# TEAM-AIOLY/OCM-VAE-SIMCA

Measured on AMD Instinct MI355X. Metric: spectra/sec SIMCA fit+Q/T² score at 1M×2048, higher is better.
Workload: dtype f32

## Files before the change

### ocm-vae-simca_amd/csrc/ocm_gram.hip

```cpp
#include <cstring>
#include <string>
#include <type_traits>
#include <vector>

#include "ocm_gram_map.h"
#include "ocm_internal.h"

namespace {

__device__ __forceinline__ float load_y(const float* __restrict__ X, int64_t ldx, int64_t r, int col, int p,
                                        const PrepArgs& pa) {
  if (pa.w == 0 && !pa.snv) return X[r * ldx + col];
  float m = 0.f, sc = 1.f;
  if (pa.snv) {
    m = pa.rowstat[2 * r];
    sc = pa.rowstat[2 * r + 1];
  }
  return ocm::prep_elem(X + r * ldx, p, col, pa, m, sc);
}


constexpr int MAXSEG = 32;

struct SegTable {
  int64_t begin[MAXSEG + 1];
  int32_t cprefix[MAXSEG + 1];
  int32_t nseg;
  int32_t chunk_rows;
};

__device__ __forceinline__ void tile_coords(int t, int nt, int& ti, int& tj) {
  ti = 0;
  while (t >= nt - ti) {
    t -= nt - ti;
    ++ti;
  }
  tj = ti + t;
}

template <int GT, int BK_>
struct GramCfg {
  static constexpr int BK = BK_;
  static constexpr int WN = GT / 64;
  static constexpr int THREADS = 2 * WN * 64;
  static constexpr int MT = GT / 64;
  static constexpr int C4 = GT / 4;
  static constexpr int RSTEP = THREADS / C4;
  static constexpr int LPP = BK / RSTEP;
};

constexpr int GATHER_MAX_CHUNK = 2048;

template <int GT, int BK_, bool VEC, bool GATHER>
__global__ __launch_bounds__(GT * 2, 2) void k_gram(
    const float* __restrict__ X, int64_t ldx, const int64_t* __restrict__ rows, int p, const float* __restrict__ shift,
    SegTable st, int nt, int ntiles, int total_wg, float* __restrict__ part, double* __restrict__ colpart) {
  using Cfg = GramCfg<GT, BK_>;
  constexpr int BK = Cfg::BK, MT = Cfg::MT, LPP = Cfg::LPP, RSTEP = Cfg::RSTEP;
  __shared__ __attribute__((aligned(16))) float lds[2][2][BK][GT];
  __shared__ int64_t ridx[GATHER ? GATHER_MAX_CHUNK : 1];

  const int b = blockIdx.x;
  const int q8 = total_wg / 8, r8 = total_wg % 8, x8 = b % 8;
  const int wg = (x8 < r8 ? x8 * (q8 + 1) : r8 * (q8 + 1) + (x8 - r8) * q8) + b / 8;
  const int chunk = wg / ntiles;
  const int tile = wg - chunk * ntiles;
  int ti, tj;
  tile_coords(tile, nt, ti, tj);
  const bool diag = (ti == tj);
  const int I = ti * GT, J = tj * GT;

  int s = 0;
  while (s + 1 < st.nseg && chunk >= st.cprefix[s + 1]) ++s;
  const int64_t r0 = st.begin[s] + (int64_t)(chunk - st.cprefix[s]) * st.chunk_rows;
  const int64_t r1 = min(r0 + (int64_t)st.chunk_rows, st.begin[s + 1]);
  const int nstage = (int)((r1 - r0 + BK - 1) / BK);

  const int tid = threadIdx.x;
  const int lane = tid & 63, wave = tid >> 6;
  const int wm = wave / Cfg::WN, wn = wave % Cfg::WN;
  if (GATHER) {
// ... 484 lines not shown
      }
    }
    if (tid < p)
      for (int r = 0; r < nr; ++r) csum += ys[r][tid];
  }
#pragma unroll
  for (int u = 0; u < MAXPT; ++u) {
    const int e = tid + 256 * u;
    if (e < npair) part[(size_t)blockIdx.x * npair + e] = acc[u];
  }
  if (tid < p) cpart[(size_t)blockIdx.x * p + tid] = csum;
}

__global__ __launch_bounds__(256) void k_gram_small_reduce(const double* __restrict__ part,
                                                           const double* __restrict__ cpart, int p, int c0, int c1,
                                                           double* __restrict__ G, double* __restrict__ colsum) {
  const int e = blockIdx.x * 256 + threadIdx.x;
  const int npair = p * (p + 1) / 2;
  if (e < npair) {
    int i = 0, rem = e;
    while (rem >= p - i) {
      rem -= p - i;
      ++i;
    }
    const int j = i + rem;
    double v = 0.0;
    for (int c = c0; c < c1; ++c) v += part[(size_t)c * npair + e];
    G[(size_t)i * p + j] = v;
    G[(size_t)j * p + i] = v;
  }
  if (e < p) {
    double v = 0.0;
    for (int c = c0; c < c1; ++c) v += cpart[(size_t)c * p + e];
    colsum[e] = v;
  }
}

typedef int i32x4 __attribute__((ext_vector_type(4)));
typedef int i32x16 __attribute__((ext_vector_type(16)));
constexpr int Q8T = 128, Q8K = 32, Q8BLK = 1536, Q8SPB = Q8BLK / Q8K;
constexpr float Q8BASE = 254.f;

struct Q8Plan {
  char* digits;
  size_t plane;
  float* scale;
  int P8;
  int nblk;
  const float* thr;
  uint32_t* flags;
  int fw;
  uint32_t* nmark;
};

constexpr float Q8TAU = 16.f;
constexpr int Q8GROUP = 32;

__device__ __forceinline__ uint32_t q8_byte(float a, int u) { return ((uint32_t)(int)a & 0xffu) << (8 * u); }

__device__ __forceinline__ uint32_t q8_pack4(float a0, float a1, float a2, float a3) {
  const uint32_t lo = __builtin_amdgcn_perm((uint32_t)(int)a1, (uint32_t)(int)a0, 0x0c0c0400u);
  const uint32_t hi = __builtin_amdgcn_perm((uint32_t)(int)a3, (uint32_t)(int)a2, 0x04000c0cu);
  return lo | hi;
}

__device__ __forceinline__ int q8_qslot(int P) { return P ^ ((P >> 3) & 7); }

constexpr int Q8QC = 32;
constexpr int Q8QS = Q8BLK / 16;
constexpr int Q8QT = Q8QS * (Q8QC / 4);
struct Q8TailLds {
  union {
    struct {
      __attribute__((aligned(16))) float wmax[Q8QS][Q8QC];
      __attribute__((aligned(16))) double wsum[Q8QS][Q8QC];
      float pmax[8][Q8QC];
      double psum[8][Q8QC];
    } r;
    __attribute__((aligned(16))) char stage[3 * Q8SPB * Q8QC * 32];
  } u;
  __attribute__((aligned(16))) float fmax_[Q8QC];
};
__device__ __forceinline__ void q8_tail(f32x4 (&v)[16], int tid, int cq, int rs, int cg0, int c0, int64_t rb,
                                        const Q8Plan& q, int chunk, int b, const SegTable& st,
                                        double* __restrict__ colblk, Q8TailLds& L, const f32x4 th) {
  constexpr int QC = Q8QC, NT = Q8QT;
  char* stage = L.u.stage;
  auto& wmax = L.u.r.wmax;
  auto& wsum = L.u.r.wsum;
  auto& pmax = L.u.r.pmax;
  auto& psum = L.u.r.psum;
  float* fmax_ = L.fmax_;
#ifdef OCM_Q8_DIAG_COPY
  (void)wsum; (void)wmax; (void)pmax; (void)psum; (void)fmax_; (void)th; (void)colblk; (void)c0;
  i32x4 w[3][4];
#pragma unroll
  for (int dg = 0; dg < 3; ++dg)
#pragma unroll
    for (int e = 0; e < 4; ++e)
#pragma unroll
      for (int k = 0; k < 4; ++k)
        w[dg][e][k] = (int)(__builtin_bit_cast(uint32_t, v[4 * k][e]) ^ __builtin_bit_cast(uint32_t, v[4 * k + 1][e]) ^
                            __builtin_bit_cast(uint32_t, v[4 * k + 2][e]) ^ __builtin_bit_cast(uint32_t, v[4 * k + 3][e])) + dg;
#else
  double cs[4] = {0.0, 0.0, 0.0, 0.0};
#pragma unroll
// ... 585 lines not shown
      const bool mi = (m >> (ty >> 3)) & 1u;
      const bool mj = (m >> (2 + (tx >> 3))) & 1u;
      if (!(mi || mj)) continue;
#pragma unroll
      for (int a = 0; a < 4; ++a) {
        const double u = yi[r][4 * ty + a];
#pragma unroll
        for (int b = 0; b < 4; ++b) acc[a][b] = fma(u, yj[r][4 * tx + b], acc[a][b]);
      }
    }
  }
  double* Gs = G + (size_t)seg * p * p;
#pragma unroll
  for (int a = 0; a < 4; ++a)
#pragma unroll
    for (int b = 0; b < 4; ++b) {
      const int gi = I + 4 * ty + a, gj = J + 4 * tx + b;
      if (gi >= p || gj >= p) continue;
      Gs[(size_t)gi * p + gj] += acc[a][b];
      if (ti != tj) Gs[(size_t)gj * p + gi] += acc[a][b];
    }
}

__global__ __launch_bounds__(256, 1) void k_gram8d(Q8Plan q, SegTable st, int nt, int ntiles, int total_wg,
                                                   int nwg, int nblocks, float* __restrict__ part) {
  __shared__ __attribute__((aligned(16))) float scl[4][2 * 64];
  __shared__ __attribute__((aligned(16))) float runl[4][4][4][64][4];

  const int wg = ocm_g8::logical_item(total_wg, blockIdx.x);
  const int chunk = wg / nwg;
  const int wave = __builtin_amdgcn_readfirstlane(threadIdx.x >> 6);
  const int bi = (wg - chunk * nwg) * 4 + wave;
  if (bi >= nblocks) return;
  int ti = -1, tj = 0, wm = 0, wn = 0;
  {
    int rem = bi;
    for (int u = 0; u < nt && ti < 0; u += ocm_g8::BAND_R)
      for (int v = u; v < nt && ti < 0; v += ocm_g8::BAND_C)
        for (int a = u; a < min(nt, u + ocm_g8::BAND_R) && ti < 0; ++a)
          for (int c = max(v, a); c < min(nt, v + ocm_g8::BAND_C); ++c) {
            const int nbk = (a == c) ? 3 : 4;
            if (rem < nbk) {
              ti = a;
              tj = c;
              wm = (a == c) ? (rem == 2) : (rem >> 1);
              wn = (a == c) ? (rem >= 1) : (rem & 1);
              break;
            }
            rem -= nbk;
          }
  }
  const int tile = ti * nt - ti * (ti - 1) / 2 + (tj - ti);
  const int I = ti * Q8T, J = tj * Q8T;
  int s = 0;
  while (s + 1 < st.nseg && chunk >= st.cprefix[s + 1]) ++s;
  const int64_t r0 = st.begin[s] + (int64_t)(chunk - st.cprefix[s]) * st.chunk_rows;
  const int64_t r1 = min(r0 + (int64_t)st.chunk_rows, st.begin[s + 1]);
  const int nb = (int)((r1 - r0 + Q8BLK - 1) / Q8BLK);
  const int nstage3 = nb * Q8SPB;
  const size_t gbase = (size_t)chunk * (st.chunk_rows / Q8K);

  const int lane = threadIdx.x & 63;
  const int l31 = lane & 31, h = lane >> 5;
  const size_t gstride = (size_t)q.P8 * 32;
  const uint32_t span = (uint32_t)((size_t)nstage3 * gstride);
  const char* cbase = q.digits + gbase * gstride;
  __amdgpu_buffer_rsrc_t ra[3], rb[3];
#pragma unroll
  for (int dg = 0; dg < 3; ++dg) {
    ra[dg] = __builtin_amdgcn_make_buffer_rsrc((void*)(cbase + dg * q.plane + (size_t)(I + wm * 64) * 32), 0, span,
                                               0x00020000);
    rb[dg] = __builtin_amdgcn_make_buffer_rsrc((void*)(cbase + dg * q.plane + (size_t)(J + wn * 64) * 32), 0, span,
                                               0x00020000);
  }
  const int voff = l31 * 32 + h * 16;
  const float* srow = q.scale + (size_t)chunk * q.nblk * q.P8 + I + wm * 64 + lane;
  const float* scol = q.scale + (size_t)chunk * q.nblk * q.P8 + J + wn * 64 + lane;

#define Q8D_LOAD(FA, FB, STG)                                                                         \
  do {                                                                                              \
    const int so_ = (STG) * (int)gstride;                                                           \
    _Pragma("unroll") for (int x_ = 0; x_ < 2; ++x_)                                                \
    _Pragma("unroll") for (int dg_ = 0; dg_ < 3; ++dg_) {                                           \
      FA[x_][dg_] = (i32x4)__builtin_amdgcn_raw_buffer_load_b128(ra[dg_], voff + x_ * 1024, so_, 0); \
      FB[x_][dg_] = (i32x4)__builtin_amdgcn_raw_buffer_load_b128(rb[dg_], voff + x_ * 1024, so_, 0); \
    }                                                                                               \
  } while (0)
  i32x16 acc1[2][2], acc2[2][2], acc3[2][2];
#pragma unroll
  for (int a = 0; a < 2; ++a)
#pragma unroll
    for (int c = 0; c < 2; ++c) {
      acc1[a][c] = i32x16{};
      acc2[a][c] = i32x16{};
      acc3[a][c] = i32x16{};
#pragma unroll
      for (int g = 0; g < 4; ++g)
        *reinterpret_cast<f32x4*>(&runl[wave][a * 2 + c][g][lane][0]) = f32x4{0.f, 0.f, 0.f, 0.f};
    }
  float SR = 0.f, SC = 0.f;
  auto flush = [&]() __attribute__((always_inline)) {
    constexpr float w2 = 1.f / 254.f, w3 = 1.f / (254.f * 254.f);
    scl[wave][lane] = SR;
    scl[wave][64 + lane] = SC;
#pragma unroll
    for (int a = 0; a < 2; ++a) {
#pragma unroll
      for (int c = 0; c < 2; ++c) {
        const float sj = scl[wave][64 + c * 32 + l31];
#pragma unroll
        for (int g = 0; g < 4; ++g) {
          const f32x4 si = *reinterpret_cast<const f32x4*>(&scl[wave][a * 32 + 8 * g + 4 * h]);
          f32x4* rp = reinterpret_cast<f32x4*>(&runl[wave][a * 2 + c][g][lane][0]);
          f32x4 rv = *rp;
#pragma unroll
          for (int e = 0; e < 4; ++e) {
            const int r = 4 * g + e;
            const float v = fmaf((float)acc3[a][c][r], w3, fmaf((float)acc2[a][c][r], w2, (float)acc1[a][c][r]));
            rv[e] = fmaf(v, si[e] * sj, rv[e]);
          }
          *rp = rv;
        }
        __builtin_amdgcn_sched_barrier(0);
      }
    }
  };
  auto step_il = [&](i32x4 (&CA)[2][3], i32x4 (&CB)[2][3], i32x4 (&NA)[2][3], i32x4 (&NB)[2][3], int stg,
                     bool z) __attribute__((always_inline)) {
    const int so_ = min(stg + 2, nstage3 - 1) * (int)gstride;
#pragma unroll
// ... 73 lines not shown
#endif
constexpr int G8P_TMAP = 2048;
template <bool SKIP>
__global__ __launch_bounds__(256, 1) void k_gram8e(Q8Plan q, SegTable st, int nt, int ntiles, int total_wg,
                                                   int nwg, int nblocks, float* __restrict__ part, int chunk0,
                                                   int map) {
  __shared__ __attribute__((aligned(16))) float scl[4][2 * 64];
  __shared__ __attribute__((aligned(16))) float runl[4][16][64][4];
  __shared__ uint16_t tmap[G8P_TMAP];

  const int noffr = ntiles - nt;
  const bool tabled = noffr <= G8P_TMAP;
  if (tabled) {
    for (int r = threadIdx.x; r < noffr; r += 256) {
      int a, c;
      ocm_g8::offdiag_tile(nt, r, a, c);
      tmap[r] = (uint16_t)(a << 8 | c);
    }
    __syncthreads();
  }
  const ocm_g8::Slot sl = ocm_g8::map_slot(map, total_wg, (int)gridDim.x, (int)blockIdx.x);
  if (sl.count == 0) return;

  const int wave = __builtin_amdgcn_readfirstlane(threadIdx.x >> 6);
  const int lane = threadIdx.x & 63;
  const int l15 = lane & 15, g4 = lane >> 4;
  constexpr int SPB = Q8BLK / 64;
  const size_t gstride = (size_t)q.P8 * 32;
  const int voff = (g4 >> 1) * (int)gstride + l15 * 32 + (g4 & 1) * 16;
  const int sstride = 2 * (int)gstride;
  const int vout = (4 * g4 * Q8T + l15) * 4;
  constexpr uint32_t OUT_SPAN = (63 * Q8T + 64) * 4;

  struct Item {
    __amdgpu_buffer_rsrc_t ra[3], rb[3];
    __amdgpu_buffer_rsrc_t rout;
    const float *srow, *scol;
    int nb, nvs;
  };
  auto setup = [&](int wg) __attribute__((always_inline)) -> Item {
    const int cl = wg / nwg, chunk = chunk0 + cl;
    ocm_g8::Block k = ocm_g8::block_of(nt, ntiles, nblocks, wg - cl * nwg, wave);
    if (k.offrank >= 0) {
      if (tabled) {
        const int v = __builtin_amdgcn_readfirstlane((int)tmap[k.offrank]);
        k.ti = v >> 8;
        k.tj = v & 255;
      } else {
        ocm_g8::offdiag_tile(nt, k.offrank, k.ti, k.tj);
      }
    }
    const int tile = ocm_g8::tile_index(nt, k.ti, k.tj);
    const int I = k.ti * Q8T + k.wm * 64, J = k.tj * Q8T + k.wn * 64;
    int s = 0;
    while (s + 1 < st.nseg && chunk >= st.cprefix[s + 1]) ++s;
    const int64_t r0 = st.begin[s] + (int64_t)(chunk - st.cprefix[s]) * st.chunk_rows;
    const int64_t r1 = min(r0 + (int64_t)st.chunk_rows, st.begin[s + 1]);
    Item it;
    it.nb = (int)((r1 - r0 + Q8BLK - 1) / Q8BLK);
    it.nvs = SKIP ? (int)((r1 - r0 + 63) / 64) : it.nb * SPB;
    const size_t gbase = (size_t)chunk * (st.chunk_rows / Q8K);
    const uint32_t span = (uint32_t)((size_t)it.nb * Q8SPB * gstride);
    const char* cbase = q.digits + gbase * gstride;
#pragma unroll
    for (int dg = 0; dg < 3; ++dg) {
      it.ra[dg] = __builtin_amdgcn_make_buffer_rsrc((void*)(cbase + dg * q.plane + (size_t)I * 32), 0, span, 0x00020000);
      it.rb[dg] = __builtin_amdgcn_make_buffer_rsrc((void*)(cbase + dg * q.plane + (size_t)J * 32), 0, span, 0x00020000);
    }
    it.srow = q.scale + (size_t)chunk * q.nblk * q.P8 + I;
    it.scol = q.scale + (size_t)chunk * q.nblk * q.P8 + J;
    float* out = part + ((size_t)chunk * ntiles + tile) * (Q8T * Q8T) + k.wm * 64 * Q8T + k.wn * 64;
    it.rout = __builtin_amdgcn_make_buffer_rsrc((void*)out, 0, k.dead ? 0u : OUT_SPAN, 0x00020000);
    return it;
  };

  i32x4 acc1[4][4], acc2[4][4], acc3[4][4];
  float SR = 0.f, SC = 0.f;
  auto flush = [&](bool first) __attribute__((always_inline)) {
    constexpr float w2 = 1.f / 254.f, w3 = 1.f / (254.f * 254.f);
    scl[wave][lane] = SR;
    scl[wave][64 + lane] = SC;
#pragma unroll
    for (int a = 0; a < 4; ++a) {
      const f32x4 si = *reinterpret_cast<const f32x4*>(&scl[wave][a * 16 + 4 * g4]);
#pragma unroll
      for (int c = 0; c < 4; ++c) {
        const float sj = scl[wave][64 + c * 16 + l15];
        f32x4* rp = reinterpret_cast<f32x4*>(&runl[wave][a * 4 + c][lane][0]);
        f32x4 rv = *rp;
        if (first) rv = f32x4{0.f, 0.f, 0.f, 0.f};
#pragma unroll
        for (int e = 0; e < 4; ++e) {
          const float v = fmaf((float)acc3[a][c][e], w3, fmaf((float)acc2[a][c][e], w2, (float)acc1[a][c][e]));
          rv[e] = fmaf(v, si[e] * sj, rv[e]);
        }
        *rp = rv;
      }
      __builtin_amdgcn_sched_barrier(0);
    }
  };
  auto load_frag = [&](i32x4 (&FA)[4][3], i32x4 (&FB)[4][3], int i, int so, const __amdgpu_buffer_rsrc_t (&da)[3],
                       const __amdgpu_buffer_rsrc_t (&db)[3]) __attribute__((always_inline)) {
    const int grp = i / 3, dg = i % 3;
    if (grp >= 1 && grp <= 4)
      FB[grp - 1][dg] = (i32x4)__builtin_amdgcn_raw_buffer_load_b128(db[dg], voff + (grp - 1) * 512, so, 0);
    else {
      const int x = grp == 0 ? 0 : grp - 4;
      FA[x][dg] = (i32x4)__builtin_amdgcn_raw_buffer_load_b128(da[dg], voff + x * 512, so, 0);
    }
  };
  auto store_sub = [&](const f32x4& pv, int i, __amdgpu_buffer_rsrc_t ro) __attribute__((always_inline)) {
    const int a = i >> 2, c = i & 3;
#pragma unroll
    for (int e = 0; e < 4; ++e)
      __builtin_amdgcn_raw_buffer_store_b32(__builtin_bit_cast(unsigned, (float)pv[e]), ro, vout,
                                            ((a * 16 + e) * Q8T + c * 16) * 4, OCM_G8E_STORE_AUX);
  };
  auto step = [&](i32x4 (&CA)[4][3], i32x4 (&CB)[4][3], i32x4 (&NA)[4][3], i32x4 (&NB)[4][3], int so,
                  const __amdgpu_buffer_rsrc_t (&da)[3], const __amdgpu_buffer_rsrc_t (&db)[3], bool z, bool bar,
                  auto tail, __amdgpu_buffer_rsrc_t ro) __attribute__((always_inline)) {
    constexpr bool TAIL = decltype(tail)::value;
    f32x4 pv = {0.f, 0.f, 0.f, 0.f};
#pragma unroll
// ... 156 lines not shown
      tab.cprefix[s - s0] = cprefix[s] - cprefix[s0];
    }
    const int64_t gchunks = cprefix[s1] - cprefix[s0];
    if (gchunks == 0) continue;
    const int64_t total = gchunks * ntiles;
    OCM_REQUIRE(total < (1LL << 31), "ocm_gram_f32: too many workgroups");
    float* pg = part + (size_t)cprefix[s0] * ntiles * GT * GT;
    double* col_g = colpart + (size_t)cprefix[s0] * nt * GT;
    ocm::TimedRegion tr(ctx, OCM_KERNEL_GRAM, st);
    dim3 grid((unsigned)total), blk(Cfg::THREADS);
#define OCM_GRAM_LAUNCH(V_, G_)                                                                                    \
  hipLaunchKernelGGL((k_gram<GT, BK, V_, G_>), grid, blk, 0, st, X, ldx, rows, p, shift, tab, nt, ntiles, (int)total, \
                     pg, col_g)
    if (split3) {
      if (rows)
        hipLaunchKernelGGL(k_gram3<true>, grid, dim3(G3THREADS), 0, st, X, ldx, rows, p, shift, tab, nt, ntiles,
                           (int)total, pg, col_g);
      else
        hipLaunchKernelGGL(k_gram3<false>, grid, dim3(G3THREADS), 0, st, X, ldx, rows, p, shift, tab, nt, ntiles,
                           (int)total, pg, col_g);
    } else if (rows) {
      if (vec) OCM_GRAM_LAUNCH(true, true); else OCM_GRAM_LAUNCH(false, true);
    } else {
      if (vec) OCM_GRAM_LAUNCH(true, false); else OCM_GRAM_LAUNCH(false, false);
    }
#undef OCM_GRAM_LAUNCH
    OCM_CHECK_LAUNCH("k_gram");
  }
  for (int s = 0; s < nseg; ++s) {
    double* Gs = G_out + (size_t)s * p * p;
    double* cs = colsum_out + (size_t)s * p;
    if (cprefix[s + 1] == cprefix[s]) {
      OCM_HIP(hipMemsetAsync(Gs, 0, (size_t)p * p * sizeof(double), st));
      OCM_HIP(hipMemsetAsync(cs, 0, (size_t)p * sizeof(double), st));
      continue;
    }
    dim3 g((GT * GT / 4 + 255) / 256, ntiles);
    hipLaunchKernelGGL(k_gram_reduce<GT>, g, dim3(256), 0, st, part, colpart, nt, ntiles, p, cprefix[s],
                       cprefix[s + 1], Gs, cs);
    OCM_CHECK_LAUNCH("k_gram_reduce");
  }
  return OCM_OK;
}

int gram_impl8(ocm_ctx* ctx, const float* X, int64_t ldx, const int64_t* rows, int64_t n, int32_t p,
               const float* shift, const int64_t* seg_offsets, int32_t nseg, double* G_out, double* colsum_out,
               hipStream_t st, int64_t chunk_rows, bool k32, const PrepArgs& pa = PrepArgs{},
               bool unguarded = false, float* xout = nullptr, int64_t ldo = 0, const float* tr_O = nullptr,
               double* tr_part = nullptr) {
  const bool prep = pa.w > 0 || pa.snv;
  const int P8 = (int)ocm::align_up((size_t)p, Q8T);
  const int nt = P8 / Q8T;
  const int ntiles = nt * (nt + 1) / 2;
  if (chunk_rows <= 0) {
    const int64_t want = std::max<int64_t>(1, (4LL * ctx->num_cus + ntiles - 1) / ntiles);
    chunk_rows = std::min<int64_t>(4096, (n + want - 1) / want);
  }
  chunk_rows = std::max<int64_t>(Q8BLK, (int64_t)ocm::align_up((size_t)chunk_rows, Q8BLK));
  std::vector<int32_t> cprefix(nseg + 1, 0);
  for (int s = 0; s < nseg; ++s) {
    const int64_t len = seg_offsets[s + 1] - seg_offsets[s];
    cprefix[s + 1] = cprefix[s] + (int32_t)((len + chunk_rows - 1) / chunk_rows);
  }
  const int64_t nchunks = cprefix[nseg];
  const int nblk = (int)(chunk_rows / Q8BLK);
  const size_t plane = (size_t)nchunks * chunk_rows * P8;
  const size_t scale_elems = (size_t)nchunks * nblk * P8;
  const size_t col_elems = (size_t)nchunks * nblk * P8;
  const size_t part_elems = (size_t)nchunks * ntiles * Q8T * Q8T;
  const int ngrp = P8 / Q8GROUP, fw = (ngrp + 31) / 32;
  const int64_t nsamp = std::min<int64_t>(n, 4096);
  const int nsplit = (int)std::min<int64_t>((nsamp + 255) / 256, 16);
  const int64_t rps = (nsamp + nsplit - 1) / nsplit;
  const int nfblk = (int)((n + FLAG_BLK - 1) / FLAG_BLK);
  const size_t guard_bytes = (size_t)P8 * 4 + (size_t)n * fw * 4 + (size_t)p * QX_BINS * 4 + (size_t)nfblk * 4 +
                             (size_t)n * 8 + 16 * 256;
  void* wsp = ocm::workspace(ctx, 3 * plane + scale_elems * 4 + col_elems * 8 + part_elems * 4 + guard_bytes +
                                      4 * 4096, st);
  if (!wsp) return OCM_ERR_NOMEM;
  ocm::Carve cv{static_cast<char*>(wsp)};
  char* digits = cv.take<char>(3 * plane);
  float* scale = cv.take<float>(scale_elems);
  double* colpart = cv.take<double>(col_elems);
  float* part = cv.take<float>(part_elems);
  float* thr = cv.take<float>(P8);
  uint32_t* flags = cv.take<uint32_t>((size_t)n * fw);
  uint32_t* xhist = cv.take<uint32_t>((size_t)p * QX_BINS);
  uint32_t* fcnt = cv.take<uint32_t>(nfblk);
  int64_t* flist = cv.take<int64_t>(n);
  uint32_t* counters = cv.take<uint32_t>(4);
  auto* host = static_cast<uint32_t*>(ocm::host_staging(ctx, 64));
  if (!host) return OCM_ERR_NOMEM;

  if (!unguarded) {
    const size_t nf = (size_t)n * fw, third = (size_t)p * QX_BINS;
    const size_t tot = nf + 4 + third;
    hipLaunchKernelGGL(k_guard_init, dim3((unsigned)std::min<size_t>((tot + 255) / 256, 4096)), dim3(256), 0, st,
                       flags, nf, counters, xhist, third, 0u);
    OCM_CHECK_LAUNCH("k_guard_init");
  }
  if (!unguarded) {
    hipLaunchKernelGGL(k_colexp_hist, dim3((p + 63) / 64, nsplit), dim3(256), 0, st, X, ldx, rows, nsamp, p, shift,
                       rps, xhist, pa);
    hipLaunchKernelGGL(k_q8_colmed, dim3((p + 3) / 4), dim3(256), 0, st, xhist, nsamp, p, thr);
    hipLaunchKernelGGL(k_q8_thresholds, dim3(1), dim3(1024), 0, st, p, P8, thr);
    OCM_CHECK_LAUNCH("k_q8_thresholds");
  }

  std::vector<SegTable> tabs;
  std::vector<int> tab_s0;
  for (int s0 = 0; s0 < nseg; s0 += MAXSEG) {
    const int s1 = std::min(nseg, s0 + MAXSEG);
    SegTable tab{};
    tab.nseg = s1 - s0;
    tab.chunk_rows = (int32_t)chunk_rows;
    for (int s = s0; s <= s1; ++s) {
      tab.begin[s - s0] = seg_offsets[s];
      tab.cprefix[s - s0] = cprefix[s] - cprefix[s0];
    }
    const int64_t gchunks = cprefix[s1] - cprefix[s0];
    if (gchunks == 0) continue;
    OCM_REQUIRE(gchunks * ntiles < (1LL << 31) && gchunks < 65536 * 1024LL, "ocm_gram_f32: too many workgroups");
    tabs.push_back(tab);
    tab_s0.push_back(s0);
  }
  auto plan_for = [&](int s0) {
    Q8Plan q{};
    q.digits = digits + (size_t)cprefix[s0] * chunk_rows * P8;
    q.plane = plane;
    q.scale = scale + (size_t)cprefix[s0] * nblk * P8;
    q.P8 = P8;
    q.nblk = nblk;
    q.thr = unguarded ? nullptr : thr;
    q.flags = flags;
    q.fw = fw;
    q.nmark = counters;
    return q;
  };
  hipStreamCaptureStatus cap = hipStreamCaptureStatusNone;
  OCM_HIP(hipStreamIsCapturing(st, &cap));
  const bool capturing = cap != hipStreamCaptureStatusNone;
  int gmap = ocm_g8::MAP_ROUND;
#ifdef OCM_EXP_SELECTORS
  if (const char* mv = getenv("OCM_GRAM8_MAP")) gmap = !strcmp(mv, "round") ? ocm_g8::MAP_ROUND : ocm_g8::MAP_RANGE;
#endif
  const int nblocks = 4 * ntiles - nt, nwg = (nblocks + 3) / 4;
  auto tab_chunks = [&](size_t t) { return (int64_t)(cprefix[tab_s0[t] + tabs[t].nseg] - cprefix[tab_s0[t]]); };

  for (size_t t = 0; t < tabs.size(); ++t) {
    const int s0 = tab_s0[t];
    const Q8Plan q = plan_for(s0);
    double* col_g = colpart + (size_t)cprefix[s0] * nblk * P8;
    const int ncg = P8 / Q8QC;
    const unsigned nrb = (unsigned)(tab_chunks(t) * nblk);
    ocm::TimedRegion tq(ctx, OCM_KERNEL_QUANT, st, !unguarded);
    if (prep) {
#define Q8P_LAUNCH(G_, H_, W_)                                                                                     \
  hipLaunchKernelGGL((k_q8_quant_prep<G_, H_, W_>), dim3(nrb * ncg), dim3(Q8QT), 0, st, X, ldx, rows, p, shift, tabs[t], \
                     q, col_g, 0, ncg, pa, xout, ldo)
      if (pa.h == 0) {
        if (rows) Q8P_LAUNCH(true, 0, false); else if (xout) Q8P_LAUNCH(false, 0, true); else Q8P_LAUNCH(false, 0, false);
      } else if (pa.h == 2) {
        if (rows) Q8P_LAUNCH(true, 2, false); else if (xout) Q8P_LAUNCH(false, 2, true); else Q8P_LAUNCH(false, 2, false);
      } else {
        if (rows) Q8P_LAUNCH(true, 7, false); else if (xout) Q8P_LAUNCH(false, 7, true); else Q8P_LAUNCH(false, 7, false);
      }
#undef Q8P_LAUNCH
    } else if (rows) {
      hipLaunchKernelGGL(k_q8_quant<true>, dim3(nrb, ncg), dim3(Q8QT), 0, st, X, ldx, rows, p, shift, tabs[t], q, col_g, 0);
    } else {
      hipLaunchKernelGGL(k_q8_quant<false>, dim3(nrb, ncg), dim3(Q8QT), 0, st, X, ldx, rows, p, shift, tabs[t], q, col_g, 0);
    }
  }
  OCM_CHECK_LAUNCH("k_q8_quant");
  hipEvent_t ev = nullptr;
  const bool readback = !capturing && !unguarded;
  if (readback) {
    OCM_HIP(hipEventCreateWithFlags(&ev, hipEventDisableTiming));
    OCM_HIP(hipMemcpyAsync(host, counters, 4, hipMemcpyDeviceToHost, st));
    OCM_HIP(hipEventRecord(ev, st));
  }
  for (size_t t = 0; t < tabs.size(); ++t) {
    const int s0 = tab_s0[t];
    const int total = (int)(tab_chunks(t) * nwg);
    const Q8Plan q = plan_for(s0);
    float* pg = part + (size_t)cprefix[s0] * ntiles * Q8T * Q8T;
    ocm::TimedRegion tr(ctx, OCM_KERNEL_GRAM, st, !unguarded);
    const dim3 pgrid((unsigned)std::min(total, std::max(ctx->num_cus, ocm_g8::NXCD)));
    if (k32)
      hipLaunchKernelGGL(k_gram8d, dim3((unsigned)total), dim3(256), 0, st, q, tabs[t], nt, ntiles, total, nwg, nblocks,
                         pg);
    else if (tr_O)
      hipLaunchKernelGGL(k_gram8e<true>, pgrid, dim3(256), 0, st, q, tabs[t], nt, ntiles, total, nwg, nblocks, pg, 0,
                         gmap);
    else
      hipLaunchKernelGGL(k_gram8e<false>, pgrid, dim3(256), 0, st, q, tabs[t], nt, ntiles, total, nwg, nblocks, pg, 0,
                         gmap);
  }
  OCM_CHECK_LAUNCH("k_gram8d/8e");
#ifdef OCM_G8E_STAMPS
  {
    unsigned long long acc[4] = {0, 0, 0, 0};
    OCM_HIP(hipStreamSynchronize(st));
    OCM_HIP(hipMemcpyFromSymbol(acc, HIP_SYMBOL(g8_stamp_acc), sizeof(acc)));
    if (!unguarded && !capturing && acc[3])
      fprintf(stderr, "G8E_STAMPS items=%llu mean_us entry_to_first=%.3f last_to_end=%.3f entry_to_end=%.3f\n",
              acc[3], 0.01 * acc[0] / acc[3], 0.01 * acc[1] / acc[3], 0.01 * acc[2] / acc[3]);
    const unsigned long long zero[4] = {0, 0, 0, 0};
    OCM_HIP(hipMemcpyToSymbol(HIP_SYMBOL(g8_stamp_acc), zero, sizeof(zero)));
  }
#endif
  if (tr_O) {
    hipLaunchKernelGGL(k_gram_trace<Q8T>, dim3(Q8T * Q8T / 4 / 256, ntiles), dim3(256), 0, st, part, nt, ntiles, p, 0,
                       cprefix[1], tr_O, tr_part);
    OCM_CHECK_LAUNCH("k_gram_trace");
    return OCM_OK;
  }
  for (int s = 0; s < nseg; ++s) {
    double* Gs = G_out + (size_t)s * p * p;
    double* cs = colsum_out + (size_t)s * p;
    if (cprefix[s + 1] == cprefix[s]) {
      OCM_HIP(hipMemsetAsync(Gs, 0, (size_t)p * p * sizeof(double), st));
      OCM_HIP(hipMemsetAsync(cs, 0, (size_t)p * sizeof(double), st));
      continue;
    }
    dim3 g((Q8T * Q8T / 4 + 255) / 256, ntiles);
    hipLaunchKernelGGL(k_gram_reduce<Q8T>, g, dim3(256), 0, st, part, colpart, nt, ntiles, p, cprefix[s],
                       cprefix[s + 1], Gs, cs, 0);
    hipLaunchKernelGGL(k_colblk_sum, dim3(P8 / 16), dim3(256), 0, st, colpart, (int64_t)cprefix[s] * nblk,
                       (int64_t)cprefix[s + 1] * nblk, P8, p, cs);
    OCM_CHECK_LAUNCH("k_colblk_sum");
    OCM_CHECK_LAUNCH("k_gram_reduce");
  }
  if (unguarded) return OCM_OK;
  if (!capturing) {
    const hipError_t e = hipEventSynchronize(ev);
    (void)hipEventDestroy(ev);
    if (e != hipSuccess) return ocm::fail(OCM_ERR_HIP, std::string("gram mark read-back: ") + hipGetErrorString(e));
    ctx->last_gram_marks = host[0];
    if (host[0] == 0) return OCM_OK;
  }
  hipLaunchKernelGGL(k_flag_count, dim3(nfblk), dim3(256), 0, st, flags, fw, n, fcnt);
  hipLaunchKernelGGL(k_flag_emit, dim3(nfblk), dim3(256), 0, st, flags, fw, n, fcnt, nfblk, flist, counters + 1);
  OCM_CHECK_LAUNCH("k_flag_emit");
  if (!capturing) {
    OCM_HIP(hipMemcpyAsync(host + 1, counters + 1, 4, hipMemcpyDeviceToHost, st));
    OCM_HIP(hipStreamSynchronize(st));
    if ((int64_t)host[1] > n / 8) return 1;
  }
  const int nt64 = (p + FX_T - 1) / FX_T;
  for (int s0 = 0; s0 < nseg; s0 += MAXSEG) {
    const int s1 = std::min(nseg, s0 + MAXSEG);
    FixSeg fs{};
    fs.nseg = s1 - s0;
    for (int s = s0; s <= s1; ++s) fs.begin[s - s0] = seg_offsets[s];
    hipLaunchKernelGGL(k_gram_fixup, dim3(nt64 * (nt64 + 1) / 2, s1 - s0), dim3(256), 0, st, X, ldx, rows, p, shift,
                       fs, flist, counters + 1, flags, fw, nt64, G_out + (size_t)s0 * p * p, pa);
  }
  OCM_CHECK_LAUNCH("k_gram_fixup");
  return OCM_OK;
}

int gram_dispatch(ocm_ctx* ctx, const float* X, int64_t ldx, const int64_t* rows, int64_t n, int32_t p,
                  const float* shift, const int64_t* seg_offsets, int32_t nseg, int32_t mode, int64_t chunk_rows,
                  double* G_out, double* colsum_out, hipStream_t st);

int gram_materialised(ocm_ctx* ctx, const float* X, int64_t ldx, const int64_t* rows, int64_t n, int32_t p,
                      const float* shift, const int64_t* seg_offsets, int32_t nseg, int32_t mode, int64_t chunk_rows,
                      const PrepArgs& pa, double* G_out, double* colsum_out, hipStream_t st) {
  float* Y = nullptr;
  OCM_HIP(hipMallocAsync(reinterpret_cast<void**>(&Y), (size_t)n * p * sizeof(float), st));
  ++ctx->prep_materialised;
  int rc = ocm::prep_apply(ctx, X, ldx, rows, n, p, pa, Y, p, st);
  if (rc == OCM_OK)
    rc = gram_dispatch(ctx, Y, p, nullptr, n, p, shift, seg_offsets, nseg, mode, chunk_rows, G_out, colsum_out, st);
  const hipError_t e = hipFreeAsync(Y, st);
  if (rc == OCM_OK && e != hipSuccess) return ocm::fail(OCM_ERR_HIP, std::string("hipFreeAsync: ") + hipGetErrorString(e));
  return rc;
}

bool prep_fused_gram(const float* X, int64_t ldx, int32_t p, int32_t mode, const PrepArgs& pa) {
// ... 182 lines not shown
```

### ocm-vae-simca_amd/csrc/ocm_gram_map.h

```cpp
#pragma once

#if defined(__HIPCC__) || defined(__CUDACC__)
#define OCM_MAP_HD __host__ __device__ inline
#else
#define OCM_MAP_HD inline
#endif

#ifndef OCM_G8_BAND_R
#define OCM_G8_BAND_R 4
#endif
#ifndef OCM_G8_BAND_C
#define OCM_G8_BAND_C 8
#endif

namespace ocm_g8 {

constexpr int BAND_R = OCM_G8_BAND_R, BAND_C = OCM_G8_BAND_C;
constexpr int NXCD = 8;

OCM_MAP_HD int imin(int a, int b) { return a < b ? a : b; }
OCM_MAP_HD int imax(int a, int b) { return a > b ? a : b; }

OCM_MAP_HD int xcd_first(int total, int x) {
  const int q8 = total / NXCD, r8 = total % NXCD;
// ... 55 lines not shown
  for (int u = 0; u < nt && ti < 0; u += BAND_R)
    for (int v = u; v < nt && ti < 0; v += BAND_C)
      for (int a = u; a < imin(nt, u + BAND_R) && ti < 0; ++a)
        for (int c = imax(v, a); c < imin(nt, v + BAND_C); ++c) {
          const int nbk = (a == c) ? 3 : 4;
          if (rem < nbk) {
            ti = a;
            tj = c;
            wm = (a == c) ? (rem == 2) : (rem >> 1);
            wn = (a == c) ? (rem >= 1) : (rem & 1);
            break;
          }
          rem -= nbk;
        }
}

struct Block {
  int bi;
  int offrank;
  int ti, tj;
  int wm, wn;
  bool dead;
};

OCM_MAP_HD Block block_of(int nt, int ntiles, int nblocks, int local, int wave) {
  Block k;
  k.bi = local * 4 + wave;
  k.dead = k.bi >= nblocks;
  if (k.dead) k.bi = nblocks - 1;
  const int noff = 4 * (ntiles - nt);
  if (k.bi < noff) {
    k.offrank = k.bi >> 2;
    k.wm = (k.bi >> 1) & 1;
    k.wn = k.bi & 1;
    k.ti = -1;
    k.tj = 0;
  } else {
    const int d = (k.bi - noff) / 3, r = (k.bi - noff) - 3 * d;
    k.offrank = -1;
    k.ti = k.tj = d;
    k.wm = (r == 2);
    k.wn = (r >= 1);
  }
  return k;
}
OCM_MAP_HD Block block_tile(int nt, int ntiles, int nblocks, int local, int wave) {
  Block k = block_of(nt, ntiles, nblocks, local, wave);
  if (k.offrank >= 0) offdiag_tile(nt, k.offrank, k.ti, k.tj);
  return k;
}

OCM_MAP_HD int tile_index(int nt, int ti, int tj) { return ti * nt - ti * (ti - 1) / 2 + (tj - ti); }

}
```

### ocm-vae-simca_amd/csrc/ocm_internal.h

```cpp
#pragma once

#include <hip/hip_runtime.h>

#include <cstdint>
#include <cstdio>
#include <string>
#include <utility>
#include <vector>

#include "ocm.h"

struct ocm_ctx {
  int device = 0;
  void* ws = nullptr;
  size_t ws_bytes = 0;
  void* ws_aux = nullptr;
  size_t ws_aux_bytes = 0;
  void* host_pinned = nullptr;
  size_t host_bytes = 0;
  int num_cus = 256;
  uint32_t last_gram_marks = 0;
  int64_t prep_materialised = 0;
  bool timing = false;
  std::vector<std::pair<hipEvent_t, hipEvent_t>> ev[OCM_TIMED_KERNELS];
  std::vector<std::pair<hipEvent_t, hipEvent_t>> ev_pool;
  hipStream_t eig_side[2] = {nullptr, nullptr};
  hipEvent_t eig_ev[7] = {nullptr, nullptr, nullptr, nullptr, nullptr, nullptr, nullptr};
  ocm_ctx* eig_sub = nullptr;
  unsigned* eig_flag = nullptr;
  unsigned eig_epoch = 0;
  int64_t eig_test_reruns = 0;
};

namespace ocm {

struct TimedRegion {
  ocm_ctx* ctx;
  int id;
  hipStream_t st;
  std::pair<hipEvent_t, hipEvent_t> pr{nullptr, nullptr};
  TimedRegion(ocm_ctx* c, int i, hipStream_t s, bool on = true) : ctx(c), id(i), st(s) {
    if (!ctx->timing || !on) return;
    if (!ctx->ev_pool.empty()) {
      pr = ctx->ev_pool.back();
      ctx->ev_pool.pop_back();
    } else {
      (void)hipEventCreate(&pr.first);
      (void)hipEventCreate(&pr.second);
    }
    (void)hipEventRecord(pr.first, st);
  }
  ~TimedRegion() {
    if (!pr.first) return;
    (void)hipEventRecord(pr.second, st);
    ctx->ev[id].push_back(pr);
  }
};

void set_error(const std::string& msg);
int fail(int code, const std::string& msg);

void* workspace(ocm_ctx* ctx, size_t bytes, hipStream_t stream);
void* workspace_aux(ocm_ctx* ctx, size_t bytes, hipStream_t stream);
void* host_staging(ocm_ctx* ctx, size_t bytes);

inline size_t align_up(size_t x, size_t a) { return (x + a - 1) / a * a; }

struct Carve {
  char* base;
  size_t off = 0;
  template <typename T>
  T* take(size_t count) {
    off = align_up(off, 256);
    T* p = reinterpret_cast<T*>(base + off);
// ... 189 lines not shown
```

### ocm-vae-simca_amd/ocm/vae_fused.py

```python
from __future__ import annotations

import ctypes

import torch

from . import _lib
from ._lib import Context, check, ptr, stream_handle

_DT = {torch.float32: 0, torch.bfloat16: 1}
LOSS_KINDS = {"bce": 0, "euclidean": 1}


def _h(dev):
    return Context.get(dev.index).handle


_BSCRATCH = {}


def _bottleneck_scratch(dev) -> torch.Tensor:
    key = dev.index
    if key not in _BSCRATCH:
        nb = int(_lib.load().ocm_vae_bottleneck_scratch_bytes())
        _BSCRATCH[key] = torch.zeros((nb + 7) // 8, dtype=torch.float64, device=dev)
# ... 298 lines not shown
        ctx.save_for_backward(x, W, y if act else None)
        return torch.nn.functional.elu(y) if act else y

    @staticmethod
    def backward(ctx, ga):
        x, W, y = ctx.saved_tensors
        ga = ga.contiguous()
        B, N = ga.shape
        if ga.dtype == torch.bfloat16 and N % 8 == 0:
            gb = torch.empty(N, dtype=ga.dtype, device=ga.device)
            gy = torch.empty_like(ga) if ctx.act else ga
            check(_lib.load().ocm_vae_act_bias_bwd(_h(ga.device), 1 if ctx.act else 0, ptr(ga),
                                                   ptr(y) if ctx.act else None, B, N, ptr(gy) if ctx.act else None,
                                                   ptr(gb), stream_handle(ga.device)), "ocm_vae_act_bias_bwd")
        else:
            gy = torch.ops.aten.elu_backward(ga, 1.0, 1.0, 1.0, False, y) if ctx.act else ga
            gb = gy.sum(0)
        gx = None
        if ctx.needs_input_grad[0]:
            gx = gemm_sk(gy, W, False) if _sk_ok(B, W.shape[1], N, gy, W) else gy.mm(W)
        gW = gy.t().mm(x) if ctx.needs_input_grad[1] else None
        return gx, gW, gb if ctx.needs_input_grad[2] else None, None


def _bias_grad(g: torch.Tensor) -> torch.Tensor:
    g = g.contiguous()
    B, N = g.shape
    if g.dtype != torch.bfloat16 or N % 8:
        return g.sum(0)
    gb = torch.empty(N, dtype=g.dtype, device=g.device)
    check(_lib.load().ocm_vae_act_bias_bwd(_h(g.device), 0, ptr(g), None, B, N, None, ptr(gb),
                                           stream_handle(g.device)), "ocm_vae_act_bias_bwd")
    return gb


class _LinearPair(torch.autograd.Function):

    @staticmethod
    def forward(ctx, x, W1, b1, W2, b2):
        ctx.save_for_backward(x, W1, W2)
        return torch.addmm(b1, x, W1.t()), torch.addmm(b2, x, W2.t())

    @staticmethod
    def backward(ctx, g1, g2):
        x, W1, W2 = ctx.saved_tensors
        g1 = x.new_zeros((x.shape[0], W1.shape[0])) if g1 is None else g1.contiguous()
        g2 = x.new_zeros((x.shape[0], W2.shape[0])) if g2 is None else g2.contiguous()
        gx = g1.mm(W1).addmm_(g2, W2) if ctx.needs_input_grad[0] else None
        return gx, g1.t().mm(x), _bias_grad(g1), g2.t().mm(x), _bias_grad(g2)


def _adjacent(a: torch.Tensor, b: torch.Tensor) -> torch.Tensor:
    if (a.is_contiguous() and b.is_contiguous() and a.dtype == b.dtype and a.shape[1:] == b.shape[1:]
            and b.data_ptr() == a.data_ptr() + a.numel() * a.element_size()):
        return torch.as_strided(a, (a.shape[0] + b.shape[0],) + tuple(a.shape[1:]), a.stride())
    return torch.cat([a, b])


class _LinearCat(torch.autograd.Function):

    @staticmethod
    def forward(ctx, x, W1, b1, W2, b2):
        Wc, bc = _adjacent(W1, W2), _adjacent(b1, b2)
        ctx.save_for_backward(x, Wc)
        ctx.n1 = W1.shape[0]
        return torch.addmm(bc, x, Wc.t())

    @staticmethod
    def backward(ctx, G):
        x, Wc = ctx.saved_tensors
        n1 = ctx.n1
        G = G.contiguous()
        gx = G.mm(Wc) if ctx.needs_input_grad[0] else None
        gW = G.t().mm(x)
        gb = _bias_grad(G)
        return gx, gW[:n1], gb[:n1], gW[n1:], gb[n1:]


def linear_cat(x: torch.Tensor, lin1: torch.nn.Linear, lin2: torch.nn.Linear) -> torch.Tensor:
    x = x.to(lin1.weight.dtype)
    return _LinearCat.apply(x, lin1.weight, lin1.bias, lin2.weight, lin2.bias)


def linear_pair(x: torch.Tensor, lin1: torch.nn.Linear, lin2: torch.nn.Linear):
    x = x.to(lin1.weight.dtype)
    return _LinearPair.apply(x, lin1.weight, lin1.bias, lin2.weight, lin2.bias)


def linear_act(x: torch.Tensor, lin: torch.nn.Linear, act: bool) -> torch.Tensor:
    return _LinearAct.apply(x.to(lin.weight.dtype), lin.weight, lin.bias, act)


def standardise(x: torch.Tensor, mean: torch.Tensor, std: torch.Tensor, dtype=torch.bfloat16) -> torch.Tensor:
    B, L = x.shape
    out = torch.empty((B, L), dtype=dtype, device=x.device)
    check(_lib.load().ocm_vae_standardise(_h(x.device), ptr(x), B, L, ptr(mean), ptr(std), _DT[dtype], ptr(out),
                                          stream_handle(x.device)), "ocm_vae_standardise")
    return out
```

Before: 60.33 million.

## Balance Gram row-block chunks across workgroups using a cost-model planner

Adds a host-side planner that, when chunk size is auto-selected and there is a single segment, picks a number of chunks N and splits the B row blocks evenly (q or q+1 blocks per chunk). The goal is less tail imbalance across CUs and a smaller partial-sum reduction in the int8 Gram kernels. Chunk offsets in the kernels now come from a balanced first-block/count formula, and the partial buffer and reduction range are sized by N. The planner relies on hardcoded timing constants and a cache-size model, and is memoized per context. A separate Python fix adds a storage-identity check before weights are aliased as adjacent.

```diff
diff --git a/ocm-vae-simca_amd/csrc/ocm_gram.hip b/ocm-vae-simca_amd/csrc/ocm_gram.hip
--- a/ocm-vae-simca_amd/csrc/ocm_gram.hip
+++ b/ocm-vae-simca_amd/csrc/ocm_gram.hip
@@ -27,6 +27,7 @@
   int32_t cprefix[MAXSEG + 1];
   int32_t nseg;
   int32_t chunk_rows;
+  int32_t bal_q, bal_r;
 };
 
 __device__ __forceinline__ void tile_coords(int t, int nt, int& ti, int& tj) {
@@ -617,6 +618,22 @@
   int fw;
   uint32_t* nmark;
 };
+
+__device__ __forceinline__ void q8_chunk_blocks(const SegTable& st, int chunk, size_t& fb, int& nb, int64_t& nrows) {
+  if (st.bal_q > 0) {
+    fb = (size_t)ocm_g8::bal_first(st.bal_q, st.bal_r, chunk);
+    nb = ocm_g8::bal_count(st.bal_q, st.bal_r, chunk);
+    nrows = (int64_t)nb * Q8BLK;
+    return;
+  }
+  int s = 0;
+  while (s + 1 < st.nseg && chunk >= st.cprefix[s + 1]) ++s;
+  const int64_t r0 = st.begin[s] + (int64_t)(chunk - st.cprefix[s]) * st.chunk_rows;
+  const int64_t r1 = min(r0 + (int64_t)st.chunk_rows, st.begin[s + 1]);
+  fb = (size_t)chunk * (st.chunk_rows / Q8BLK);
+  nb = (int)((r1 - r0 + Q8BLK - 1) / Q8BLK);
+  nrows = r1 - r0;
+}
 
 constexpr float Q8TAU = 16.f;
 constexpr int Q8GROUP = 32;
@@ -1308,13 +1325,12 @@
   }
   const int tile = ti * nt - ti * (ti - 1) / 2 + (tj - ti);
   const int I = ti * Q8T, J = tj * Q8T;
-  int s = 0;
-  while (s + 1 < st.nseg && chunk >= st.cprefix[s + 1]) ++s;
-  const int64_t r0 = st.begin[s] + (int64_t)(chunk - st.cprefix[s]) * st.chunk_rows;
-  const int64_t r1 = min(r0 + (int64_t)st.chunk_rows, st.begin[s + 1]);
-  const int nb = (int)((r1 - r0 + Q8BLK - 1) / Q8BLK);
+  size_t fb;
+  int nb;
+  int64_t nrows;
+  q8_chunk_blocks(st, chunk, fb, nb, nrows);
   const int nstage3 = nb * Q8SPB;
-  const size_t gbase = (size_t)chunk * (st.chunk_rows / Q8K);
+  const size_t gbase = fb * Q8SPB;
 
   const int lane = threadIdx.x & 63;
   const int l31 = lane & 31, h = lane >> 5;
@@ -1330,8 +1346,8 @@
                                                0x00020000);
   }
   const int voff = l31 * 32 + h * 16;
-  const float* srow = q.scale + (size_t)chunk * q.nblk * q.P8 + I + wm * 64 + lane;
-  const float* scol = q.scale + (size_t)chunk * q.nblk * q.P8 + J + wn * 64 + lane;
+  const float* srow = q.scale + fb * q.P8 + I + wm * 64 + lane;
+  const float* scol = q.scale + fb * q.P8 + J + wn * 64 + lane;
 
 #define Q8D_LOAD(FA, FB, STG)                                                                         \
   do {                                                                                              \
@@ -1511,14 +1527,12 @@
     }
     const int tile = ocm_g8::tile_index(nt, k.ti, k.tj);
     const int I = k.ti * Q8T + k.wm * 64, J = k.tj * Q8T + k.wn * 64;
-    int s = 0;
-    while (s + 1 < st.nseg && chunk >= st.cprefix[s + 1]) ++s;
-    const int64_t r0 = st.begin[s] + (int64_t)(chunk - st.cprefix[s]) * st.chunk_rows;
-    const int64_t r1 = min(r0 + (int64_t)st.chunk_rows, st.begin[s + 1]);
     Item it;
-    it.nb = (int)((r1 - r0 + Q8BLK - 1) / Q8BLK);
-    it.nvs = SKIP ? (int)((r1 - r0 + 63) / 64) : it.nb * SPB;
-    const size_t gbase = (size_t)chunk * (st.chunk_rows / Q8K);
+    size_t fb;
+    int64_t nrows;
+    q8_chunk_blocks(st, chunk, fb, it.nb, nrows);
+    it.nvs = SKIP ? (int)((nrows + 63) / 64) : it.nb * SPB;
+    const size_t gbase = fb * Q8SPB;
     const uint32_t span = (uint32_t)((size_t)it.nb * Q8SPB * gstride);
     const char* cbase = q.digits + gbase * gstride;
 #pragma unroll
@@ -1526,8 +1540,8 @@
       it.ra[dg] = __builtin_amdgcn_make_buffer_rsrc((void*)(cbase + dg * q.plane + (size_t)I * 32), 0, span, 0x00020000);
       it.rb[dg] = __builtin_amdgcn_make_buffer_rsrc((void*)(cbase + dg * q.plane + (size_t)J * 32), 0, span, 0x00020000);
     }
-    it.srow = q.scale + (size_t)chunk * q.nblk * q.P8 + I;
-    it.scol = q.scale + (size_t)chunk * q.nblk * q.P8 + J;
+    it.srow = q.scale + fb * q.P8 + I;
+    it.scol = q.scale + fb * q.P8 + J;
     float* out = part + ((size_t)chunk * ntiles + tile) * (Q8T * Q8T) + k.wm * 64 * Q8T + k.wn * 64;
     it.rout = __builtin_amdgcn_make_buffer_rsrc((void*)out, 0, k.dead ? 0u : OUT_SPAN, 0x00020000);
     return it;
@@ -1790,10 +1804,21 @@
   const int P8 = (int)ocm::align_up((size_t)p, Q8T);
   const int nt = P8 / Q8T;
   const int ntiles = nt * (nt + 1) / 2;
+  const int nblocks = 4 * ntiles - nt, nwg = (nblocks + 3) / 4;
+  const int64_t B = (n + Q8BLK - 1) / Q8BLK;
+  const bool can_balance = nseg == 1 && !rows && !tr_O && B > 0 && B * Q8BLK < (1LL << 31);
+  int nbal = 0;
+  if (chunk_rows < 0 && can_balance) nbal = (int)std::min<int64_t>(-chunk_rows, B);
   if (chunk_rows <= 0) {
+    const bool planned = chunk_rows == 0 && can_balance;
     const int64_t want = std::max<int64_t>(1, (4LL * ctx->num_cus + ntiles - 1) / ntiles);
     chunk_rows = std::min<int64_t>(4096, (n + want - 1) / want);
-  }
+    if (planned) {
+      const int cb = (int)(std::max<int64_t>(Q8BLK, (int64_t)ocm::align_up((size_t)chunk_rows, Q8BLK)) / Q8BLK);
+      nbal = ctx->gram_plans.lookup((int)B, cb, nwg, ntiles, ctx->num_cus);
+    }
+  }
+  if (nbal > 0) chunk_rows = B * Q8BLK;
   chunk_rows = std::max<int64_t>(Q8BLK, (int64_t)ocm::align_up((size_t)chunk_rows, Q8BLK));
   std::vector<int32_t> cprefix(nseg + 1, 0);
   for (int s = 0; s < nseg; ++s) {
@@ -1805,7 +1830,7 @@
   const size_t plane = (size_t)nchunks * chunk_rows * P8;
   const size_t scale_elems = (size_t)nchunks * nblk * P8;
   const size_t col_elems = (size_t)nchunks * nblk * P8;
-  const size_t part_elems = (size_t)nchunks * ntiles * Q8T * Q8T;
+  const size_t part_elems = (size_t)(nbal > 0 ? nbal : nchunks) * ntiles * Q8T * Q8T;
   const int ngrp = P8 / Q8GROUP, fw = (ngrp + 31) / 32;
   const int64_t nsamp = std::min<int64_t>(n, 4096);
   const int nsplit = (int)std::min<int64_t>((nsamp + 255) / 256, 16);
@@ -1858,7 +1883,8 @@
     }
     const int64_t gchunks = cprefix[s1] - cprefix[s0];
     if (gchunks == 0) continue;
-    OCM_REQUIRE(gchunks * ntiles < (1LL << 31) && gchunks < 65536 * 1024LL, "ocm_gram_f32: too many workgroups");
+    OCM_REQUIRE(gchunks * ntiles < (1LL << 31) && gchunks < 65536 * 1024LL && (int64_t)nbal * ntiles < (1LL << 31),
+                "ocm_gram_f32: too many workgroups");
     tabs.push_back(tab);
     tab_s0.push_back(s0);
   }
@@ -1882,7 +1908,6 @@
 #ifdef OCM_EXP_SELECTORS
   if (const char* mv = getenv("OCM_GRAM8_MAP")) gmap = !strcmp(mv, "round") ? ocm_g8::MAP_ROUND : ocm_g8::MAP_RANGE;
 #endif
-  const int nblocks = 4 * ntiles - nt, nwg = (nblocks + 3) / 4;
   auto tab_chunks = [&](size_t t) { return (int64_t)(cprefix[tab_s0[t] + tabs[t].nseg] - cprefix[tab_s0[t]]); };
 
   for (size_t t = 0; t < tabs.size(); ++t) {
@@ -1920,19 +1945,24 @@
   }
   for (size_t t = 0; t < tabs.size(); ++t) {
     const int s0 = tab_s0[t];
-    const int total = (int)(tab_chunks(t) * nwg);
+    const int total = (int)((nbal > 0 ? nbal : tab_chunks(t)) * nwg);
     const Q8Plan q = plan_for(s0);
+    SegTable gtab = tabs[t];
+    if (nbal > 0) {
+      gtab.bal_q = (int32_t)(B / nbal);
+      gtab.bal_r = (int32_t)(B % nbal);
+    }
     float* pg = part + (size_t)cprefix[s0] * ntiles * Q8T * Q8T;
     ocm::TimedRegion tr(ctx, OCM_KERNEL_GRAM, st, !unguarded);
-    const dim3 pgrid((unsigned)std::min(total, std::max(ctx->num_cus, ocm_g8::NXCD)));
+    const dim3 pgrid((unsigned)ocm_g8::launch_grid(total, ctx->num_cus));
     if (k32)
-      hipLaunchKernelGGL(k_gram8d, dim3((unsigned)total), dim3(256), 0, st, q, tabs[t], nt, ntiles, total, nwg, nblocks,
+      hipLaunchKernelGGL(k_gram8d, dim3((unsigned)total), dim3(256), 0, st, q, gtab, nt, ntiles, total, nwg, nblocks,
                          pg);
     else if (tr_O)
-      hipLaunchKernelGGL(k_gram8e<true>, pgrid, dim3(256), 0, st, q, tabs[t], nt, ntiles, total, nwg, nblocks, pg, 0,
+      hipLaunchKernelGGL(k_gram8e<true>, pgrid, dim3(256), 0, st, q, gtab, nt, ntiles, total, nwg, nblocks, pg, 0,
                          gmap);
     else
-      hipLaunchKernelGGL(k_gram8e<false>, pgrid, dim3(256), 0, st, q, tabs[t], nt, ntiles, total, nwg, nblocks, pg, 0,
+      hipLaunchKernelGGL(k_gram8e<false>, pgrid, dim3(256), 0, st, q, gtab, nt, ntiles, total, nwg, nblocks, pg, 0,
                          gmap);
   }
   OCM_CHECK_LAUNCH("k_gram8d/8e");
@@ -1963,8 +1993,8 @@
       continue;
     }
     dim3 g((Q8T * Q8T / 4 + 255) / 256, ntiles);
-    hipLaunchKernelGGL(k_gram_reduce<Q8T>, g, dim3(256), 0, st, part, colpart, nt, ntiles, p, cprefix[s],
-                       cprefix[s + 1], Gs, cs, 0);
+    hipLaunchKernelGGL(k_gram_reduce<Q8T>, g, dim3(256), 0, st, part, colpart, nt, ntiles, p,
+                       nbal > 0 ? 0 : cprefix[s], nbal > 0 ? nbal : cprefix[s + 1], Gs, cs, 0);
     hipLaunchKernelGGL(k_colblk_sum, dim3(P8 / 16), dim3(256), 0, st, colpart, (int64_t)cprefix[s] * nblk,
                        (int64_t)cprefix[s + 1] * nblk, P8, p, cs);
     OCM_CHECK_LAUNCH("k_colblk_sum");
diff --git a/ocm-vae-simca_amd/csrc/ocm_gram_map.h b/ocm-vae-simca_amd/csrc/ocm_gram_map.h
--- a/ocm-vae-simca_amd/csrc/ocm_gram_map.h
+++ b/ocm-vae-simca_amd/csrc/ocm_gram_map.h
@@ -131,4 +131,80 @@
 
 OCM_MAP_HD int tile_index(int nt, int ti, int tj) { return ti * nt - ti * (ti - 1) / 2 + (tj - ti); }
 
-}
+OCM_MAP_HD int bal_first(int q, int r, int c) { return c * q + imin(c, r); }
+OCM_MAP_HD int bal_count(int q, int r, int c) { return q + (c < r ? 1 : 0); }
+
+constexpr int PLAN_MAX_BLOCKS = 12;
+constexpr double PLAN_T_FIX_US = 2.8, PLAN_T_BLK_US = 25.7, PLAN_REDUCE_BYTES_PER_US = 5.9e6;
+constexpr double PLAN_CACHE_BYTES = 256.0 * 1024 * 1024, PLAN_CACHE_FILL = 0.75;
+constexpr int PLAN_BLOCK_ROWS = 1536, PLAN_TILE_COLS = 128;
+
+OCM_MAP_HD int launch_grid(int total, int cus) { return imin(total, imax(cus, NXCD)); }
+
+inline double plan_cost(int nl, int bl, int ns, int bs, int nwg, int ntiles, int cus) {
+  const long long total_ll = (long long)(nl + ns) * nwg;
+  if (total_ll <= 0 || total_ll >= (1LL << 31)) return 1e300;
+  const int total = (int)total_ll, grid = launch_grid(total, cus);
+  const long long nlong_items = (long long)nl * nwg;
+  double span = 0.0;
+  for (int b = 0; b < grid; ++b) {
+    const Slot sl = round_slot(total, grid, b);
+    long long cl = sl.first < nlong_items ? (nlong_items - sl.first - 1) / grid + 1 : 0;
+    if (cl > sl.count) cl = sl.count;
+    const double t = sl.count * PLAN_T_FIX_US + PLAN_T_BLK_US * ((double)cl * bl + (double)(sl.count - cl) * bs);
+    if (t > span) span = t;
+  }
+  return span + (double)(nl + ns) * ntiles * 65536.0 / PLAN_REDUCE_BYTES_PER_US;
+}
+inline double plan_cost_balanced(int B, int N, int nwg, int ntiles, int cus) {
+  return plan_cost(B % N, B / N + 1, N - B % N, B / N, nwg, ntiles, cus);
+}
+inline double plan_cost_uniform(int B, int cb, int nwg, int ntiles, int cus) {
+  const int C = (B + cb - 1) / cb;
+  return plan_cost(C - 1, cb, 1, B - (C - 1) * cb, nwg, ntiles, cus);
+}
+
+inline int plan_max_blocks(int nwg, int ntiles, int cus) {
+  int nt = 1;
+  while (nt * (nt + 1) / 2 < ntiles) ++nt;
+  const double block_bytes = 3.0 * PLAN_BLOCK_ROWS * PLAN_TILE_COLS * nt;
+  const int live = (imax(cus, NXCD) + nwg - 1) / nwg + 1;
+  const double fit = PLAN_CACHE_BYTES * PLAN_CACHE_FILL / (live * block_bytes);
+  return fit >= PLAN_MAX_BLOCKS ? PLAN_MAX_BLOCKS : imax(1, (int)fit);
+}
+
+inline int plan_chunks(int B, int cb_uniform, int nwg, int ntiles, int cus) {
+  if (B <= 3) return 0;
+  double best = plan_cost_uniform(B, cb_uniform, nwg, ntiles, cus);
+  int bestN = 0;
+  const int maxb = plan_max_blocks(nwg, ntiles, cus);
+  for (int N = (B + maxb - 1) / maxb; N <= B; ++N) {
+    const double c = plan_cost_balanced(B, N, nwg, ntiles, cus);
+    if (c < best) {
+      best = c;
+      bestN = N;
+    }
+  }
+  return bestN;
+}
+
+struct PlanMemo {
+  static constexpr int CAP = 16;
+  struct Entry {
+    int B, nwg, grid, cb, N;
+  };
+  Entry e[CAP];
+  int used = 0, next = 0;
+  int lookup(int B, int cb_uniform, int nwg, int ntiles, int cus) {
+    const int grid = imax(cus, NXCD);
+    for (int i = 0; i < used; ++i)
+      if (e[i].B == B && e[i].nwg == nwg && e[i].grid == grid && e[i].cb == cb_uniform) return e[i].N;
+    const int N = plan_chunks(B, cb_uniform, nwg, ntiles, cus);
+    e[next] = Entry{B, nwg, grid, cb_uniform, N};
+    next = (next + 1) % CAP;
+    if (used < CAP) ++used;
+    return N;
+  }
+};
+
+}
diff --git a/ocm-vae-simca_amd/csrc/ocm_internal.h b/ocm-vae-simca_amd/csrc/ocm_internal.h
--- a/ocm-vae-simca_amd/csrc/ocm_internal.h
+++ b/ocm-vae-simca_amd/csrc/ocm_internal.h
@@ -9,6 +9,7 @@
 #include <vector>
 
 #include "ocm.h"
+#include "ocm_gram_map.h"
 
 struct ocm_ctx {
   int device = 0;
@@ -20,6 +21,7 @@
   size_t host_bytes = 0;
   int num_cus = 256;
   uint32_t last_gram_marks = 0;
+  ocm_g8::PlanMemo gram_plans;
   int64_t prep_materialised = 0;
   bool timing = false;
   std::vector<std::pair<hipEvent_t, hipEvent_t>> ev[OCM_TIMED_KERNELS];
diff --git a/ocm-vae-simca_amd/ocm/vae_fused.py b/ocm-vae-simca_amd/ocm/vae_fused.py
--- a/ocm-vae-simca_amd/ocm/vae_fused.py
+++ b/ocm-vae-simca_amd/ocm/vae_fused.py
@@ -374,7 +374,8 @@
 
 def _adjacent(a: torch.Tensor, b: torch.Tensor) -> torch.Tensor:
     if (a.is_contiguous() and b.is_contiguous() and a.dtype == b.dtype and a.shape[1:] == b.shape[1:]
-            and b.data_ptr() == a.data_ptr() + a.numel() * a.element_size()):
+            and b.data_ptr() == a.data_ptr() + a.numel() * a.element_size()
+            and a.untyped_storage().data_ptr() == b.untyped_storage().data_ptr()):
         return torch.as_strided(a, (a.shape[0] + b.shape[0],) + tuple(a.shape[1:]), a.stride())
     return torch.cat([a, b])
 
```

After: 61.66 million (median of 6 runs). +2.2%, better.
